# Neuroprosthetics-Lab/nejm-brain-to-text

Hardware: AMD Instinct MI355X
Metric: GRU+CTC train sentences/sec (higher is better)
Workload: dtype f32; 1 GPU; BASELINE.json configs[1]: 5-layer GRU-512 + CTC, synthetic [B=64,T=500,F=512] -> 41 phonemes, fp32, full training step incl. on-GPU augmentation, clip and AdamW; global_batch=64, rows_per_rank=64, seq_len=500, parallelism=dp1, world_size_seen=1, gru_mode=1

## Files before the change

### nejm-brain-to-text_amd/csrc/gemm.hip

```cpp
#include "common.h"
#include "gemm_args.h"

namespace b2t {

using f32x16 = float __attribute__((ext_vector_type(16)));
using f32x4 = float __attribute__((ext_vector_type(4)));

#ifndef B2T_GEMM_BK
#define B2T_GEMM_BK 16
#endif
#ifndef B2T_GEMM_OCC
#define B2T_GEMM_OCC 3
#endif
constexpr int BM = 128, BN = 128, BKT = B2T_GEMM_BK;
constexpr int NLD = BKT / 8;
constexpr int TPR = BKT / 4;
constexpr int RPP = 256 / TPR;
template <bool KC> struct Pitch { static constexpr int v = KC ? 129 : 132; };
constexpr int PITCH_MAX = 132;

template <bool KC>
__device__ __forceinline__ void load_full(const float* __restrict__ P, const long long (&roff)[NLD], int mcl, int k0,
                                          long long s0, long long s1, int div, float4 (&v)[NLD], int tid) {
#pragma unroll
  for (int r = 0; r < NLD; ++r) {
    if constexpr (KC) {
      v[r] = *reinterpret_cast<const float4*>(P + roff[r] + k0 + (tid % TPR) * 4);
    } else {
      v[r] = *reinterpret_cast<const float4*>(P + rowoff(k0 + (tid >> 5) + 8 * r, s0, s1, div) + mcl);
    }
  }
}

template <bool KC>
__device__ __forceinline__ void load_tail(const float* __restrict__ P, const long long (&roff)[NLD], int ext_m,
                                          int base_m, int k0, int Kend, long long s0, long long s1, int div,
                                          float4 (&v)[NLD], int tid) {
#pragma unroll
  for (int r = 0; r < NLD; ++r) {
    float4 o = make_float4(0.f, 0.f, 0.f, 0.f);
    if constexpr (KC) {
      const int row = base_m + tid / TPR + RPP * r;
      const int k = k0 + (tid % TPR) * 4;
      if (row < ext_m) {
        const float* p = P + roff[r] + k;
        if (k < Kend) o.x = p[0];
        if (k + 1 < Kend) o.y = p[1];
        if (k + 2 < Kend) o.z = p[2];
        if (k + 3 < Kend) o.w = p[3];
      }
    } else {
      const int k = k0 + (tid >> 5) + 8 * r;
      const int m = base_m + (tid & 31) * 4;
      if (k < Kend) {
        const float* p = P + rowoff(k, s0, s1, div) + m;
        if (m < ext_m) o.x = p[0];
        if (m + 1 < ext_m) o.y = p[1];
        if (m + 2 < ext_m) o.z = p[2];
        if (m + 3 < ext_m) o.w = p[3];
      }
    }
    v[r] = o;
  }
}

template <bool KC>
__device__ __forceinline__ void store_tile(float* __restrict__ S, const float4 (&v)[NLD], int tid) {
  constexpr int PITCH = Pitch<KC>::v;
#pragma unroll
  for (int r = 0; r < NLD; ++r) {
    if constexpr (KC) {
      const int row = tid / TPR + RPP * r;
      const int k = (tid % TPR) * 4;
      S[(k + 0) * PITCH + row] = v[r].x;
      S[(k + 1) * PITCH + row] = v[r].y;
      S[(k + 2) * PITCH + row] = v[r].z;
      S[(k + 3) * PITCH + row] = v[r].w;
    } else {
      const int k = (tid >> 5) + 8 * r;
      const int m = (tid & 31) * 4;
      *reinterpret_cast<float4*>(&S[k * PITCH + m]) = v[r];
    }
  }
}

__device__ __forceinline__ float4 load_f4_sc1(const float* base_uniform, unsigned byte_off) {
  using u32x4 = unsigned int __attribute__((ext_vector_type(4)));
  __amdgpu_buffer_rsrc_t rsrc = __builtin_amdgcn_make_buffer_rsrc(const_cast<float*>(base_uniform), 0, 0x7fffffff, 0x00020000);
  const u32x4 v = __builtin_amdgcn_raw_buffer_load_b128(rsrc, byte_off, 0, 16);
  return make_float4(__uint_as_float(v.x), __uint_as_float(v.y), __uint_as_float(v.z), __uint_as_float(v.w));
}

template <bool AKC, bool BKC>
__global__ __launch_bounds__(256, B2T_GEMM_OCC) void gemm_f32_kernel(GemmArgs g) {
  __shared__ __attribute__((aligned(16))) float smem[2 * 2 * BKT * PITCH_MAX];
  constexpr int PA = Pitch<AKC>::v, PB = Pitch<BKC>::v;
  float* As = smem;
  float* Bs = smem + 2 * BKT * PITCH_MAX;

  const int tid = threadIdx.x;
  const int lane = tid & 63, wave = tid >> 6;
  const int wm = wave >> 1, wn = wave & 1;
  int z = blockIdx.z / g.splitk;
  int ks = blockIdx.z - z * g.splitk;
  int m0, n0;
  {
    const int gx = (g.N + BN - 1) / BN, nwg = gridDim.x;
    int tile;
    if (g.ks_xcd) {
      const int lin = blockIdx.x + nwg * blockIdx.z, xcd = lin & 7, j = lin >> 3;
      ks = xcd + 8 * (j / nwg); tile = j % nwg; z = 0;
    } else {
      const int b = blockIdx.x, xcd = b & 7, qq = nwg >> 3, rr = nwg & 7;
      tile = (xcd < rr ? xcd * (qq + 1) : rr * (qq + 1) + (xcd - rr) * qq) + (b >> 3);
    }
    m0 = (tile / gx) * BM; n0 = (tile % gx) * BN;
  }

  const float* A = g.A + (long long)z * g.a_sz;
  const int zb = g.b_zmap ? g.b_zmap[z] : z;
  const float* B = g.B + (long long)zb * g.b_sz;
  const float* bias = (g.bias && ks == 0) ? g.bias + (long long)zb * g.bias_sz : nullptr;
  float* C = g.C + (long long)z * g.c_sz + (long long)ks * g.c_ks;

  long long roffA[NLD], roffB[NLD];
#pragma unroll
  for (int r = 0; r < NLD; ++r) {
    const int ra_ = m0 + tid / TPR + RPP * r, rb_ = n0 + tid / TPR + RPP * r;
    roffA[r] = AKC ? rowoff(ra_ < g.M ? ra_ : g.M - 1, g.a_s0, g.a_s1, g.a_div) : 0;
    roffB[r] = BKC ? rowoff(rb_ < g.N ? rb_ : g.N - 1, g.b_s0, g.b_s1, g.b_div) : 0;
  }
  const int mclA = min(m0 + (tid & 31) * 4, ((g.M + 3) & ~3) - 4);
  const int mclB = min(n0 + (tid & 31) * 4, ((g.N + 3) & ~3) - 4);

  f32x16 acc[2][2];
#pragma unroll
  for (int i = 0; i < 2; ++i)
#pragma unroll
    for (int j = 0; j < 2; ++j)
#pragma unroll
      for (int e = 0; e < 16; ++e) acc[i][j][e] = 0.f;

  const int kb = ks * g.kchunk;
  const int K = min(g.K, kb + g.kchunk);
  const int nk = (K - kb + BKT - 1) / BKT;
  const int nfull = (K - kb) / BKT;
  float4 ra[NLD], rb[NLD];

  auto fetch = [&](int kt) {
    const int k0 = kb + kt * BKT;
    const float* Ag = A + ((g.a_brk > 0 && (AKC ? k0 : m0) >= g.a_brk) ? g.a_gap : 0);
    if (kt < nfull) {
      load_full<AKC>(Ag, roffA, mclA, k0, g.a_s0, g.a_s1, g.a_div, ra, tid);
      load_full<BKC>(B, roffB, mclB, k0, g.b_s0, g.b_s1, g.b_div, rb, tid);
    } else {
      load_tail<AKC>(Ag, roffA, g.M, m0, k0, K, g.a_s0, g.a_s1, g.a_div, ra, tid);
      load_tail<BKC>(B, roffB, g.N, n0, k0, K, g.b_s0, g.b_s1, g.b_div, rb, tid);
    }
  };
  const bool do_sum = !AKC && g.a_sum != nullptr && n0 == 0;
  float4 asum = make_float4(0.f, 0.f, 0.f, 0.f);
  auto add_a = [&]() {
    if constexpr (!AKC) {
      if (do_sum) {
#pragma unroll
        for (int r = 0; r < NLD; ++r) { asum.x += ra[r].x; asum.y += ra[r].y; asum.z += ra[r].z; asum.w += ra[r].w; }
      }
    }
  };
  fetch(0);
  add_a();
  store_tile<AKC>(As, ra, tid);
  store_tile<BKC>(Bs, rb, tid);
  __syncthreads();

  const int lk = lane >> 5, li = lane & 31;
  int cur = 0;
  for (int kt = 0; kt < nk; ++kt) {
    const bool more = kt + 1 < nk;
    if (more) fetch(kt + 1);
    const float* as = As + cur * BKT * PA + wm * 64 + li + lk * PA;
    const float* bs = Bs + cur * BKT * PB + wn * 64 + li + lk * PB;
    float a0 = as[0], a1 = as[32], b0 = bs[0], b1 = bs[32];
#pragma unroll
    for (int kk = 0; kk < BKT; kk += 2) {
      float na0 = 0.f, na1 = 0.f, nb0 = 0.f, nb1 = 0.f;
      if (kk + 2 < BKT) {
        na0 = as[(kk + 2) * PA]; na1 = as[(kk + 2) * PA + 32];
        nb0 = bs[(kk + 2) * PB]; nb1 = bs[(kk + 2) * PB + 32];
      }
      acc[0][0] = __builtin_amdgcn_mfma_f32_32x32x2f32(a0, b0, acc[0][0], 0, 0, 0);
      acc[0][1] = __builtin_amdgcn_mfma_f32_32x32x2f32(a0, b1, acc[0][1], 0, 0, 0);
      acc[1][0] = __builtin_amdgcn_mfma_f32_32x32x2f32(a1, b0, acc[1][0], 0, 0, 0);
      acc[1][1] = __builtin_amdgcn_mfma_f32_32x32x2f32(a1, b1, acc[1][1], 0, 0, 0);
      a0 = na0; a1 = na1; b0 = nb0; b1 = nb1;
    }
    if (more) {
      add_a();
      store_tile<AKC>(As + (cur ^ 1) * BKT * PA, ra, tid);
      store_tile<BKC>(Bs + (cur ^ 1) * BKT * PB, rb, tid);
    }
    __syncthreads();
    cur ^= 1;
  }

  if constexpr (!AKC) {
    if (do_sum) {
      float4* red = reinterpret_cast<float4*>(smem);
      red[tid] = asum;
      __syncthreads();
      if (tid < 32) {
        float4 t = red[tid];
#pragma unroll
        for (int gq = 1; gq < 8; ++gq) { const float4 u = red[gq * 32 + tid]; t.x += u.x; t.y += u.y; t.z += u.z; t.w += u.w; }
        float* o = g.a_sum + ((long long)z * g.splitk + ks) * g.a_sum_ks;
        const int m = m0 + tid * 4;
        if (m < g.M) o[m] = t.x;
        if (m + 1 < g.M) o[m + 1] = t.y;
        if (m + 2 < g.M) o[m + 2] = t.z;
        if (m + 3 < g.M) o[m + 3] = t.w;
      }
    }
  }
#pragma unroll
  for (int i = 0; i < 2; ++i) {
#pragma unroll
    for (int j = 0; j < 2; ++j) {
      const int col = n0 + wn * 64 + j * 32 + li;
      if (col >= g.N) continue;
      const float bv = bias ? bias[col] : 0.f;
#pragma unroll
      for (int e = 0; e < 16; ++e) {
        const int row = m0 + wm * 64 + i * 32 + (e & 3) + 8 * (e >> 2) + 4 * lk;
        if (row < g.M) {
          float v = acc[i][j][e] + bv;
          if (g.epilogue == 1) v = v / (1.0f + fabsf(v));
          const long long coff = rowoff(row, g.c_s0, g.c_s1, g.c_div) + col;
          if (g.epilogue == 2) { const float a = 1.0f - fabsf(g.ep_aux[(long long)z * g.c_sz + coff]); v *= a * a; }
          float* p = C + coff;
          if (g.accumulate) v += *p;
          if (g.ks_cnt) __hip_atomic_store(p, v, __ATOMIC_RELAXED, __HIP_MEMORY_SCOPE_AGENT);
          else *p = v;
        }
      }
    }
  }
  if (g.ks_cnt) {
    asm volatile("s_waitcnt vmcnt(0)" ::: "memory");
    __syncthreads();
    int* flag = reinterpret_cast<int*>(smem);
    const int gx = (g.N + BN - 1) / BN, tile_id = (m0 / BM) * gx + n0 / BN;
    if (tid == 0) {
      const unsigned old = __hip_atomic_fetch_add(g.ks_cnt + tile_id, 1u, __ATOMIC_RELAXED, __HIP_MEMORY_SCOPE_AGENT);
      const int last = old == (unsigned)g.splitk - 1u;
      if (last) __hip_atomic_store(g.ks_cnt + tile_id, 0u, __ATOMIC_RELAXED, __HIP_MEMORY_SCOPE_AGENT);
      flag[0] = last;
    }
    __syncthreads();
    if (flag[0]) {
      for (int idx = tid; idx < BM * (BN / 4); idx += 256) {
        const int r = m0 + idx / (BN / 4), cc = n0 + (idx % (BN / 4)) * 4;
        if (r >= g.M || cc >= g.N) continue;
        const long long e = (long long)r * g.N + cc;
        float4 acc = make_float4(0.f, 0.f, 0.f, 0.f);
        if (g.ks_acc) acc = *reinterpret_cast<const float4*>(g.ks_out + e);
        for (int sl = 0; sl < g.splitk; ++sl) {
          const float4 v = load_f4_sc1(g.C + (long long)sl * g.c_ks, (unsigned)(e * 4));
          acc.x += v.x; acc.y += v.y; acc.z += v.z; acc.w += v.w;
        }
        *reinterpret_cast<float4*>(g.ks_out + e) = acc;
      }
    }
  }
}


template <int MT, bool BKC>
__global__ __launch_bounds__(512) void gemm_skinny_kernel(GemmArgs g) {
  __shared__ float red[8][MT][4][64];
  const int tid = threadIdx.x, lane = tid & 63, wave = tid >> 6;
  const int j = lane & 15, q = lane >> 4;
  const int n0 = blockIdx.x * 16;
  const int z = blockIdx.y, zb = g.b_zmap ? g.b_zmap[z] : z;
  g.A += (long long)z * g.a_sz; g.B += (long long)zb * g.b_sz; g.C += (long long)z * g.c_sz;
  if (g.bias) g.bias += (long long)zb * g.bias_sz;
  const int ncol = n0 + j < g.N ? n0 + j : g.N - 1;
  const float* brow = BKC ? g.B + rowoff(ncol, g.b_s0, g.b_s1, g.b_div) + 4 * q : g.B + ncol;
  const float* arow[MT];
#pragma unroll
  for (int mt = 0; mt < MT; ++mt) {
    const int r = 16 * mt + j;
    arow[mt] = g.A + rowoff(r < g.M ? r : g.M - 1, g.a_s0, g.a_s1, g.a_div) + 4 * q;
  }
  f32x4 acc[MT];
#pragma unroll
  for (int mt = 0; mt < MT; ++mt) acc[mt] = f32x4{0.f, 0.f, 0.f, 0.f};
  const int nchunk = g.K / 16;
  for (int c0 = wave * 4; c0 < nchunk; c0 += 32) {
    float4 bw[4], av[4][MT];
#pragma unroll
    for (int u = 0; u < 4; ++u) {
      const int k = (c0 + u < nchunk ? c0 + u : c0) * 16;
      if constexpr (BKC) {
        bw[u] = *reinterpret_cast<const float4*>(brow + k);
      } else {
        const int kq = k + 4 * q;
        bw[u] = make_float4(brow[rowoff(kq, g.b_s0, g.b_s1, g.b_div)], brow[rowoff(kq + 1, g.b_s0, g.b_s1, g.b_div)],
                            brow[rowoff(kq + 2, g.b_s0, g.b_s1, g.b_div)], brow[rowoff(kq + 3, g.b_s0, g.b_s1, g.b_div)]);
      }
#pragma unroll
      for (int mt = 0; mt < MT; ++mt) av[u][mt] = *reinterpret_cast<const float4*>(arow[mt] + k);
    }
#pragma unroll
    for (int u = 0; u < 4; ++u) {
      if (c0 + u < nchunk) {
#pragma unroll
        for (int mt = 0; mt < MT; ++mt) {
          acc[mt] = __builtin_amdgcn_mfma_f32_16x16x4f32(av[u][mt].x, bw[u].x, acc[mt], 0, 0, 0);
          acc[mt] = __builtin_amdgcn_mfma_f32_16x16x4f32(av[u][mt].y, bw[u].y, acc[mt], 0, 0, 0);
          acc[mt] = __builtin_amdgcn_mfma_f32_16x16x4f32(av[u][mt].z, bw[u].z, acc[mt], 0, 0, 0);
          acc[mt] = __builtin_amdgcn_mfma_f32_16x16x4f32(av[u][mt].w, bw[u].w, acc[mt], 0, 0, 0);
        }
      }
    }
  }
#pragma unroll
  for (int mt = 0; mt < MT; ++mt)
#pragma unroll
    for (int e = 0; e < 4; ++e) red[wave][mt][e][lane] = acc[mt][e];
  __syncthreads();
  for (int idx = tid; idx < MT * 4 * 64; idx += 512) {
    const int l = idx & 63, e = (idx >> 6) & 3, mt = idx >> 8;
    const float v0 = (red[0][mt][e][l] + red[1][mt][e][l]) + (red[2][mt][e][l] + red[3][mt][e][l]);
    const float v1 = (red[4][mt][e][l] + red[5][mt][e][l]) + (red[6][mt][e][l] + red[7][mt][e][l]);
    const int row = 16 * mt + 4 * (l >> 4) + e, col = n0 + (l & 15);
    if (row < g.M && col < g.N) {
      float v = v0 + v1 + (g.bias ? g.bias[col] : 0.f);
      if (g.epilogue == 1) v = v / (1.0f + fabsf(v));
      float* p = g.C + rowoff(row, g.c_s0, g.c_s1, g.c_div) + col;
      if (g.accumulate) v += *p;
      *p = v;
    }
  }
}

}

extern "C" int b2t_gemm_f32(const b2t_gemm_desc* d, void* stream) {
  using namespace b2t;
  B2T_REQUIRE(d != nullptr, "b2t_gemm_f32: null descriptor");
  B2T_REQUIRE(d->M > 0 && d->N > 0 && d->K > 0 && d->Z > 0, "b2t_gemm_f32: bad shape M=%d N=%d K=%d Z=%d",
              d->M, d->N, d->K, d->Z);
  B2T_REQUIRE(((uintptr_t)d->A & 15) == 0 && ((uintptr_t)d->B & 15) == 0, "b2t_gemm_f32: A/B must be 16-byte aligned");
  B2T_REQUIRE((d->a_s0 % 4) == 0 && (d->a_s1 % 4) == 0 && (d->a_sz % 4) == 0 && (d->b_s0 % 4) == 0 &&
                  (d->b_s1 % 4) == 0 && (d->b_sz % 4) == 0,
              "b2t_gemm_f32: A/B strides must be multiples of 4 elements");
  B2T_REQUIRE(d->a_sum == nullptr || !d->a_kcontig, "b2t_gemm_f32: a_sum goes with an m-contiguous A (a_kcontig = 0)");
  B2T_REQUIRE(d->ks_counters == nullptr || (d->splitk > 1 && d->Z == 1 && (d->N % 4) == 0 && d->ks_out != nullptr && ((uintptr_t)d->ks_out & 15) == 0 &&
                                            (long long)d->M * d->N * 4 < (1ll << 31)),
              "b2t_gemm_f32: the in-kernel slab reduction needs splitk > 1, Z = 1, N %% 4 == 0 and a 16-byte aligned ks_out");
  GemmArgs g;
  { int rc = fill_gemm_args(d, g, BKT, BM, "b2t_gemm_f32"); if (rc) return rc; }
  dim3 grid(((d->N + BN - 1) / BN) * ((d->M + BM - 1) / BM), 1, d->Z * g.splitk), block(256);
  { static const bool off = getenv("B2T_GEMM_KS_XCD") && atoi(getenv("B2T_GEMM_KS_XCD")) == 0; g.ks_xcd = !off && d->Z == 1 && g.splitk >= 8 && (g.splitk & 7) == 0; }
  hipStream_t s = as_stream(stream);
  if (d->M <= 64 && d->splitk >= 0 && g.splitk == 1 && d->a_kcontig && (d->K % 16) == 0 && d->a_brk == 0 && d->epilogue != 2) {
    const dim3 sg((d->N + 15) / 16, d->Z), sb(512);
#define B2T_SKINNY(MT)                                                                                  \
    do {                                                                                                \
      if (d->b_kcontig) hipLaunchKernelGGL((gemm_skinny_kernel<MT, true>), sg, sb, 0, s, g);              \
      else hipLaunchKernelGGL((gemm_skinny_kernel<MT, false>), sg, sb, 0, s, g);                          \
    } while (0)
    if (d->M <= 16) B2T_SKINNY(1);
    else if (d->M <= 32) B2T_SKINNY(2);
    else if (d->M <= 48) B2T_SKINNY(3);
    else B2T_SKINNY(4);
#undef B2T_SKINNY
    B2T_CHECK_LAUNCH("b2t_gemm_f32 (skinny)");
    return 0;
  }
  if (d->a_kcontig && d->b_kcontig) hipLaunchKernelGGL((gemm_f32_kernel<true, true>), grid, block, 0, s, g);
  else if (d->a_kcontig && !d->b_kcontig) hipLaunchKernelGGL((gemm_f32_kernel<true, false>), grid, block, 0, s, g);
  else if (!d->a_kcontig && d->b_kcontig) hipLaunchKernelGGL((gemm_f32_kernel<false, true>), grid, block, 0, s, g);
  else hipLaunchKernelGGL((gemm_f32_kernel<false, false>), grid, block, 0, s, g);
  B2T_CHECK_LAUNCH("b2t_gemm_f32");
  return 0;
}
```

### nejm-brain-to-text_amd/csrc/gemm_args.h

```cpp
#pragma once
#include "common.h"

namespace b2t {

struct GemmArgs {
  const float* A; const float* B; float* C; const float* bias;
  int M, N, K;
  long long a_s0, a_s1; int a_div; long long a_sz;
  long long b_s0, b_s1; int b_div; long long b_sz;
  long long c_s0, c_s1; int c_div; long long c_sz;
  const int* b_zmap; long long bias_sz;
  int epilogue; int accumulate;
  int splitk; int kchunk; long long c_ks;
  int a_brk; int a_gap;
  const float* ep_aux;
  float* a_sum; long long a_sum_ks;
  unsigned* ks_cnt; float* ks_out; int ks_acc;
  int ks_xcd;
  int tile_gm;
};

__device__ __forceinline__ long long rowoff(int i, long long s0, long long s1, int div) {
  return div > 0 ? (long long)(i / div) * s1 + (long long)(i % div) * s0 : (long long)i * s0;
}

inline int fill_gemm_args(const b2t_gemm_desc* d, GemmArgs& g, int bk, int bm, const char* name) {
  g.A = d->A; g.B = d->B; g.C = d->C; g.bias = d->bias;
  g.M = d->M; g.N = d->N; g.K = d->K;
  g.a_s0 = d->a_s0; g.a_s1 = d->a_s1; g.a_div = d->a_div; g.a_sz = d->a_sz;
  g.b_s0 = d->b_s0; g.b_s1 = d->b_s1; g.b_div = d->b_div; g.b_sz = d->b_sz;
  g.c_s0 = d->c_s0; g.c_s1 = d->c_s1; g.c_div = d->c_div; g.c_sz = d->c_sz;
  g.b_zmap = d->b_zmap; g.bias_sz = d->bias_sz; g.epilogue = d->epilogue; g.accumulate = d->accumulate;
  g.splitk = d->splitk > 1 ? d->splitk : 1;
  B2T_REQUIRE(g.splitk == 1 || (d->epilogue == 0 && d->accumulate == 0),
              "%s: split-K slabs cannot carry an epilogue/accumulate (reduce them with b2t_colsum_f32)", name);
  g.kchunk = ((d->K + g.splitk - 1) / g.splitk + bk - 1) / bk * bk;
  g.c_ks = d->c_ks;
  g.a_brk = d->a_brk; g.a_gap = d->a_gap;
  g.ep_aux = d->ep_aux;
  g.a_sum = d->a_sum; g.a_sum_ks = d->a_sum_ks;
  g.ks_xcd = 0; g.tile_gm = 1;
  g.ks_cnt = d->ks_counters; g.ks_out = d->ks_out; g.ks_acc = d->ks_accumulate;
  B2T_REQUIRE(d->epilogue != 2 || d->ep_aux != nullptr, "%s: epilogue 2 needs ep_aux", name);
  B2T_REQUIRE(d->a_brk == 0 || (d->a_brk > 0 && d->a_gap % 4 == 0 &&
                                (d->a_kcontig ? d->a_brk % bk == 0 : (d->a_brk % bm == 0 && d->M % bm == 0))),
              "%s: a_brk must be a multiple of the tile extent (%d along k, %d along m with M %% %d == 0), a_gap of 4", name, bk, bm, bm);
  return 0;
}

struct PackDrop { float p; unsigned long long seed; long long elem0; float* dup; };
size_t gemm_bf16p_operand_bytes(int rows, int K);
int gemm_bf16p_pack(const b2t_gemm_desc* d, int which, void* out, hipStream_t s, const PackDrop* drop = nullptr);
int gemm_bf16p_run(const b2t_gemm_desc* d, const void* Ap_pre, const void* Bp_pre, void* ws, size_t ws_bytes, hipStream_t s, const PackDrop* dropA = nullptr);

}
```

Baseline: 3432 sentences/s.

## Add steady-state GEMM k-loop with buffer loads and explicit MFMA/LDS interleaving

Adds a specialized steady-state main loop for the fp32 MFMA GEMM covering full k-tiles. It uses raw buffer loads with precomputed per-lane offsets, an incrementally advanced tile offset, precomputed LDS staging addresses, and sched_group_barrier hints to interleave global loads, LDS reads, MFMAs and LDS writes. The goal is to cut per-iteration address arithmetic and bounds checks and to improve overlap of memory and matrix ops. In exchange it adds code complexity and a gating check that operand extents fit in 32-bit byte offsets, and it relies on fields such as nfull, kb, roffA and mclA that are defined in parts of the kernel not shown.

```diff
diff --git a/nejm-brain-to-text_amd/csrc/gemm.hip b/nejm-brain-to-text_amd/csrc/gemm.hip
--- a/nejm-brain-to-text_amd/csrc/gemm.hip
+++ b/nejm-brain-to-text_amd/csrc/gemm.hip
@@ -65,23 +65,30 @@
 }
 
 template <bool KC>
-__device__ __forceinline__ void store_tile(float* __restrict__ S, const float4 (&v)[NLD], int tid) {
+__device__ __forceinline__ int stage_off(int tid) {
+  constexpr int PITCH = Pitch<KC>::v;
+  return KC ? (tid % TPR) * 4 * PITCH + tid / TPR : (tid >> 5) * PITCH + (tid & 31) * 4;
+}
+
+template <bool KC>
+__device__ __forceinline__ void store_staged(float* __restrict__ S, const float4 (&v)[NLD]) {
   constexpr int PITCH = Pitch<KC>::v;
 #pragma unroll
   for (int r = 0; r < NLD; ++r) {
     if constexpr (KC) {
-      const int row = tid / TPR + RPP * r;
-      const int k = (tid % TPR) * 4;
-      S[(k + 0) * PITCH + row] = v[r].x;
-      S[(k + 1) * PITCH + row] = v[r].y;
-      S[(k + 2) * PITCH + row] = v[r].z;
-      S[(k + 3) * PITCH + row] = v[r].w;
+      S[0 * PITCH + RPP * r] = v[r].x;
+      S[1 * PITCH + RPP * r] = v[r].y;
+      S[2 * PITCH + RPP * r] = v[r].z;
+      S[3 * PITCH + RPP * r] = v[r].w;
     } else {
-      const int k = (tid >> 5) + 8 * r;
-      const int m = (tid & 31) * 4;
-      *reinterpret_cast<float4*>(&S[k * PITCH + m]) = v[r];
-    }
-  }
+      *reinterpret_cast<float4*>(&S[8 * r * PITCH]) = v[r];
+    }
+  }
+}
+
+template <bool KC>
+__device__ __forceinline__ void store_tile(float* __restrict__ S, const float4 (&v)[NLD], int tid) {
+  store_staged<KC>(S + stage_off<KC>(tid), v);
 }
 
 __device__ __forceinline__ float4 load_f4_sc1(const float* base_uniform, unsigned byte_off) {
@@ -89,6 +96,90 @@
   __amdgpu_buffer_rsrc_t rsrc = __builtin_amdgcn_make_buffer_rsrc(const_cast<float*>(base_uniform), 0, 0x7fffffff, 0x00020000);
   const u32x4 v = __builtin_amdgcn_raw_buffer_load_b128(rsrc, byte_off, 0, 16);
   return make_float4(__uint_as_float(v.x), __uint_as_float(v.y), __uint_as_float(v.z), __uint_as_float(v.w));
+}
+
+
+template <bool KC> struct TileWalk {
+  unsigned off;
+  unsigned step, wrap;
+  int rem, div;
+  __device__ __forceinline__ TileWalk(int k0, long long s0, long long s1, int dv) {
+    if constexpr (KC) {
+      off = 4u * (unsigned)k0; step = 4u * BKT; wrap = 0; rem = 0; div = BKT;
+    } else {
+      off = 4u * (unsigned)rowoff(k0, s0, s1, dv);
+      step = 4u * BKT * (unsigned)s0; wrap = dv > 0 ? 4u * (unsigned)(s1 - dv * s0) : 0u; rem = dv > 0 ? k0 % dv : 0; div = dv > 0 ? dv : BKT;
+    }
+  }
+  __device__ __forceinline__ void next() {
+    off += step;
+    if constexpr (!KC) { rem += BKT; if (rem == div) { rem = 0; off += wrap; } }
+  }
+};
+
+__device__ __forceinline__ __amdgpu_buffer_rsrc_t operand_rsrc(const float* base_uniform) {
+  return __builtin_amdgcn_make_buffer_rsrc(const_cast<float*>(base_uniform), 0, 0x7fffffff, 0x00020000);
+}
+__device__ __forceinline__ float4 load_f4_tile(__amdgpu_buffer_rsrc_t rsrc, unsigned lane_off, unsigned tile_off_uniform) {
+  using u32x4 = unsigned int __attribute__((ext_vector_type(4)));
+  const u32x4 v = __builtin_amdgcn_raw_buffer_load_b128(rsrc, lane_off, tile_off_uniform, 0);
+  return make_float4(__uint_as_float(v.x), __uint_as_float(v.y), __uint_as_float(v.z), __uint_as_float(v.w));
+}
+
+template <int PA, int PB>
+__device__ __forceinline__ void mfma_tile(const float* as_, const float* bs_, f32x16 (&acc)[2][2]) {
+  using lds_frag = const volatile __attribute__((address_space(3))) float*;
+  lds_frag as = (lds_frag)as_;
+  lds_frag bs = (lds_frag)bs_;
+  float a0 = as[0], a1 = as[32], b0 = bs[0], b1 = bs[32];
+#pragma unroll
+  for (int kk = 0; kk < BKT; kk += 2) {
+    float na0 = 0.f, na1 = 0.f, nb0 = 0.f, nb1 = 0.f;
+    if (kk + 2 < BKT) {
+      na0 = as[(kk + 2) * PA]; na1 = as[(kk + 2) * PA + 32];
+      nb0 = bs[(kk + 2) * PB]; nb1 = bs[(kk + 2) * PB + 32];
+    }
+    acc[0][0] = __builtin_amdgcn_mfma_f32_32x32x2f32(a0, b0, acc[0][0], 0, 0, 0);
+    acc[0][1] = __builtin_amdgcn_mfma_f32_32x32x2f32(a0, b1, acc[0][1], 0, 0, 0);
+    acc[1][0] = __builtin_amdgcn_mfma_f32_32x32x2f32(a1, b0, acc[1][0], 0, 0, 0);
+    acc[1][1] = __builtin_amdgcn_mfma_f32_32x32x2f32(a1, b1, acc[1][1], 0, 0, 0);
+    a0 = na0; a1 = na1; b0 = nb0; b1 = nb1;
+  }
+}
+
+template <bool AKC, bool BKC, bool SUM>
+__device__ __forceinline__ void steady_loop(int ntiles, const float* A, const float* B, TileWalk<AKC> wa, TileWalk<BKC> wb, int to_brk,
+                                            unsigned gap_bytes, const unsigned (&offA)[NLD], const unsigned (&offB)[NLD], float* sa,
+                                            float* sb, const float* fa, const float* fb, float4 (&ra)[NLD], float4 (&rb)[NLD], f32x16 (&acc)[2][2],
+                                            float4& asum) {
+  constexpr int PA = Pitch<AKC>::v, PB = Pitch<BKC>::v;
+  const __amdgpu_buffer_rsrc_t ra_rsrc = operand_rsrc(A), rb_rsrc = operand_rsrc(B);
+  int ca = 0, cb = 0;
+  for (int kt = 0; kt < ntiles; ++kt) {
+    asm volatile("; gemm_f32 steady k-loop sum=%0" ::"n"(SUM ? 1 : 0));
+#pragma unroll
+    for (int r = 0; r < NLD; ++r) { ra[r] = load_f4_tile(ra_rsrc, offA[r], wa.off); rb[r] = load_f4_tile(rb_rsrc, offB[r], wb.off); }
+    wa.next(); wb.next();
+    if constexpr (AKC) { to_brk -= BKT; if (to_brk == 0) wa.off += gap_bytes; }
+    mfma_tile<PA, PB>(fa + ca, fb + cb, acc);
+    if constexpr (SUM) {
+#pragma unroll
+      for (int r = 0; r < NLD; ++r) { asum.x += ra[r].x; asum.y += ra[r].y; asum.z += ra[r].z; asum.w += ra[r].w; }
+    }
+    ca = BKT * PA - ca; cb = BKT * PB - cb;
+    store_staged<AKC>(sa + ca, ra);
+    store_staged<BKC>(sb + cb, rb);
+    __builtin_amdgcn_sched_group_barrier(0x020, 2 * NLD, 0);
+    __builtin_amdgcn_sched_group_barrier(0x100, 4, 0);
+#pragma unroll
+    for (int kk = 0; kk < BKT; kk += 2) {
+      if (kk + 2 < BKT) __builtin_amdgcn_sched_group_barrier(0x100, 4, 0);
+      __builtin_amdgcn_sched_group_barrier(0x008, 4, 0);
+    }
+    if constexpr (SUM) __builtin_amdgcn_sched_group_barrier(0x002, 4 * NLD, 0);
+    __builtin_amdgcn_sched_group_barrier(0x200, 8 * NLD, 0);
+    __syncthreads();
+  }
 }
 
 template <bool AKC, bool BKC>
@@ -175,8 +266,35 @@
   __syncthreads();
 
   const int lk = lane >> 5, li = lane & 31;
-  int cur = 0;
-  for (int kt = 0; kt < nk; ++kt) {
+  int cur = 0, kt = 0;
+  if (g.steady && nfull >= 2) {
+    unsigned offA[NLD], offB[NLD];
+#pragma unroll
+    for (int r = 0; r < NLD; ++r) {
+      offA[r] = 4u * (unsigned)(AKC ? roffA[r] + (tid % TPR) * 4 : ((tid >> 5) + 8 * r) * g.a_s0 + mclA);
+      offB[r] = 4u * (unsigned)(BKC ? roffB[r] + (tid % TPR) * 4 : ((tid >> 5) + 8 * r) * g.b_s0 + mclB);
+    }
+    const int k1 = kb + BKT;
+    const bool gap1 = g.a_brk > 0 && (AKC ? k1 : m0) >= g.a_brk;
+    TileWalk<AKC> wa(k1, g.a_s0, g.a_s1, g.a_div);
+    const TileWalk<BKC> wb(k1, g.b_s0, g.b_s1, g.b_div);
+    if (gap1) wa.off += 4u * (unsigned)g.a_gap;
+    const int to_brk = AKC && g.a_brk > 0 ? g.a_brk - k1 : -1;
+    float* sa = As + stage_off<AKC>(tid);
+    float* sb = Bs + stage_off<BKC>(tid);
+    const float* fa = As + wm * 64 + li + lk * PA;
+    const float* fb = Bs + wn * 64 + li + lk * PB;
+    bool summed = false;
+    if constexpr (!AKC) {
+      if (do_sum) {
+        steady_loop<AKC, BKC, true>(nfull - 1, A, B, wa, wb, to_brk, 4u * (unsigned)g.a_gap, offA, offB, sa, sb, fa, fb, ra, rb, acc, asum);
+        summed = true;
+      }
+    }
+    if (!summed) steady_loop<AKC, BKC, false>(nfull - 1, A, B, wa, wb, to_brk, 4u * (unsigned)g.a_gap, offA, offB, sa, sb, fa, fb, ra, rb, acc, asum);
+    kt = nfull - 1; cur = kt & 1;
+  }
+  for (; kt < nk; ++kt) {
     const bool more = kt + 1 < nk;
     if (more) fetch(kt + 1);
     const float* as = As + cur * BKT * PA + wm * 64 + li + lk * PA;
@@ -345,6 +463,8 @@
 }
 
 }
+
+extern "C" int b2t_gemm_f32_steady(const b2t_gemm_desc* d) { return d != nullptr && b2t::gemm_steady_ok(d, b2t::BKT); }
 
 extern "C" int b2t_gemm_f32(const b2t_gemm_desc* d, void* stream) {
   using namespace b2t;
@@ -363,6 +483,7 @@
   { int rc = fill_gemm_args(d, g, BKT, BM, "b2t_gemm_f32"); if (rc) return rc; }
   dim3 grid(((d->N + BN - 1) / BN) * ((d->M + BM - 1) / BM), 1, d->Z * g.splitk), block(256);
   { static const bool off = getenv("B2T_GEMM_KS_XCD") && atoi(getenv("B2T_GEMM_KS_XCD")) == 0; g.ks_xcd = !off && d->Z == 1 && g.splitk >= 8 && (g.splitk & 7) == 0; }
+  g.steady = gemm_steady_ok(d, BKT);
   hipStream_t s = as_stream(stream);
   if (d->M <= 64 && d->splitk >= 0 && g.splitk == 1 && d->a_kcontig && (d->K % 16) == 0 && d->a_brk == 0 && d->epilogue != 2) {
     const dim3 sg((d->N + 15) / 16, d->Z), sb(512);
diff --git a/nejm-brain-to-text_amd/csrc/gemm_args.h b/nejm-brain-to-text_amd/csrc/gemm_args.h
--- a/nejm-brain-to-text_amd/csrc/gemm_args.h
+++ b/nejm-brain-to-text_amd/csrc/gemm_args.h
@@ -18,6 +18,7 @@
   unsigned* ks_cnt; float* ks_out; int ks_acc;
   int ks_xcd;
   int tile_gm;
+  int steady;
 };
 
 __device__ __forceinline__ long long rowoff(int i, long long s0, long long s1, int div) {
@@ -39,7 +40,7 @@
   g.a_brk = d->a_brk; g.a_gap = d->a_gap;
   g.ep_aux = d->ep_aux;
   g.a_sum = d->a_sum; g.a_sum_ks = d->a_sum_ks;
-  g.ks_xcd = 0; g.tile_gm = 1;
+  g.ks_xcd = 0; g.tile_gm = 1; g.steady = 0;
   g.ks_cnt = d->ks_counters; g.ks_out = d->ks_out; g.ks_acc = d->ks_accumulate;
   B2T_REQUIRE(d->epilogue != 2 || d->ep_aux != nullptr, "%s: epilogue 2 needs ep_aux", name);
   B2T_REQUIRE(d->a_brk == 0 || (d->a_brk > 0 && d->a_gap % 4 == 0 &&
@@ -48,6 +49,21 @@
   return 0;
 }
 
+inline int gemm_steady_ok(const b2t_gemm_desc* d, int bk) {
+  auto rows_ext = [](long long n, long long s0, long long s1, int div) {
+    return div > 0 ? ((n - 1) / div) * s1 + (long long)(div - 1) * s0 : (n - 1) * s0;
+  };
+  auto operand_ok = [&](bool kc, long long ext_m, long long s0, long long s1, int div, long long gap) {
+    if (s0 < 0 || s1 < 0 || div < 0 || gap < 0) return false;
+    if (!kc && div > 0 && div % bk != 0) return false;
+    const long long rows = kc ? ext_m : (long long)d->K, run = kc ? (long long)d->K : ((ext_m + 3) & ~3ll);
+    const long long ext = rows_ext(rows, s0, s1, div) + run + (gap > 0 ? gap : 0);
+    return ext * 4 < (1ll << 31);
+  };
+  return operand_ok(d->a_kcontig != 0, d->M, d->a_s0, d->a_s1, d->a_div, d->a_brk > 0 ? d->a_gap : 0) &&
+         operand_ok(d->b_kcontig != 0, d->N, d->b_s0, d->b_s1, d->b_div, 0);
+}
+
 struct PackDrop { float p; unsigned long long seed; long long elem0; float* dup; };
 size_t gemm_bf16p_operand_bytes(int rows, int K);
 int gemm_bf16p_pack(const b2t_gemm_desc* d, int which, void* out, hipStream_t s, const PackDrop* drop = nullptr);
```

Measured after the change: 3508 sentences/s, median of 6. +2.2%, better.
